# tanhuajie/Pytorch-RT1-for-Distributed-Training

Hardware: AMD Instinct MI355X
Metric: train samples/sec (whole node), RT-1 Language-Table, 1/2/4/8 MI355X (higher is better)
Workload: dtype bf16; 1 GPU; model=RT-1 (FiLM-EfficientNet-B3 + TokenLearner-8 + 8-layer transformer, 35.3M params), global_batch=128, batch_per_gpu=128, seq_len=6, parallelism=dp1, backend=hip, hipgraph=True, step=graph, graph_segments=1, tuned_library_gemms=True, full=False

## Files before the change

pytorch_rt1_for_distributed_training_amd/csrc/bindings.cpp:

```cpp
#include <algorithm>
#include <cmath>
#include <cstdlib>

#include <torch/extension.h>
#include <c10/hip/HIPStream.h>
#include <hip/hip_runtime.h>

#include "rt1_kernels.h"

namespace {

hipStream_t cur_stream() { return c10::hip::getCurrentHIPStream().stream(); }

bool sync_check() {
    static const bool on = [] {
        const char* e = std::getenv("RT1_SYNC_CHECK");
        return e != nullptr && *e != '\0' && *e != '0';
    }();
    return on;
}

void check_launch(int err, const char* what) {
    TORCH_CHECK(err == 0, what, ": HIP launch failed: ", hipGetErrorString((hipError_t)err));
    if (sync_check()) {
// ... 1522 lines not shown
          py::arg("dst"), py::arg("src"), py::arg("splits"), py::arg("sstride"));
    m.def("multi_add_", &multi_add_, "dst[i] += src[i] for many fp32 tensors, 128 per launch");
    m.def("colsum", &colsum_py, "deterministic fixed-order sum over dim 0 (fp32/bf16 in, fp32 out)");
    m.def("frame_pool", &frame_pool);
    m.def("block_tail", &block_tail);
    m.def("tail_bwd_reduce", &tail_bwd_reduce);
    m.def("stem_fwd", &stem_fwd);
    m.def("stem_bwd_weight", &stem_bwd_weight, py::arg("img"), py::arg("shift"), py::arg("dy"), py::arg("max_blocks"),
          py::arg("bn_x") = py::none(), py::arg("scale") = py::none(), py::arg("shift_bn") = py::none(),
          py::arg("mean") = py::none(), py::arg("rstd") = py::none(), py::arg("gamma") = py::none(),
          py::arg("mdz") = py::none(), py::arg("mdzx") = py::none());
    m.def("attn_fwd", &attn_fwd, py::arg("qkv"), py::arg("L"), py::arg("Kimg"), py::arg("scale"), py::arg("drop_p"),
          py::arg("seed"), py::arg("seed_dev") = py::none());
    m.def("se_bn_bwd_reduce", &se_bn_bwd_reduce);
    m.def("proj_bwd", &proj_bwd, "project-conv backward sums + dWp from (dy3, y2) per frame (skinny blocks)");
    m.def("proj_bwd_supported", &proj_bwd_supported);
    m.def("attn_keepmask", &attn_keepmask, py::arg("BH"), py::arg("S"), py::arg("drop_p"), py::arg("seed"),
          py::arg("like"), py::arg("seed_dev") = py::none());
    m.def("attn_bwd", &attn_bwd, py::arg("qkv"), py::arg("out"), py::arg("dout"), py::arg("lse"), py::arg("L"),
          py::arg("Kimg"), py::arg("scale"), py::arg("drop_p"), py::arg("seed"), py::arg("seed_dev") = py::none());
    m.def("tf_ln_fwd", &tf_ln_fwd);
    m.def("tf_ln_bwd", &tf_ln_bwd, py::arg("dy"), py::arg("x"), py::arg("mu"), py::arg("rs"), py::arg("g"),
          py::arg("dres") = py::none(), py::arg("want_bf") = false);
    m.def("tf_resid", &tf_resid, py::arg("x"), py::arg("a"), py::arg("bias"), py::arg("p"), py::arg("seed"),
          py::arg("seed_dev") = py::none(), py::arg("lg") = py::none(), py::arg("lb") = py::none(), py::arg("eps") = 1e-6);
    m.def("tf_drop_bwd", &tf_drop_bwd, py::arg("dout"), py::arg("p"), py::arg("seed"), py::arg("seed_dev") = py::none());
    m.def("pw_gemm_supported", &pw_gemm_supported);
    m.def("pw_stats_supported", &pw_stats_supported);
    m.def("add_scaled_", &add_scaled_);
    m.def("pw_bwd_supported", &pw_bwd_supported);
    m.def("pw_bwd", &pw_bwd);
    m.def("pw_bwd_z", &pw_bwd_z);
    m.def("pw_z_prep", &pw_z_prep);
    m.def("pw_gemm_bnbwd_supported", &pw_gemm_bnbwd_supported);
    m.def("pw_gemm_bnbwd", &pw_gemm_bnbwd);
    m.def("pw_tall_tail", &pw_tall_tail, py::arg("A"), py::arg("W"), py::arg("A2"), py::arg("W2"), py::arg("bias"),
          py::arg("res") = py::none(), py::arg("rmul") = py::none(), py::arg("rhw") = 1);
    m.def("pw_z_finish", &pw_z_finish);
    rt1comm::register_comm(m);
    rt1head::register_head(m);
    m.def("pw_gemm", &pw_gemm, py::arg("A"), py::arg("B"), py::arg("max_blocks"), py::arg("stats") = false,
          py::arg("scale") = py::none(), py::arg("shift") = py::none(), py::arg("gate") = py::none(),
          py::arg("hw") = 0, py::arg("store_operand") = false);
}
```

pytorch_rt1_for_distributed_training_amd/csrc/kernels/pwbwd.hip:

```cpp
#include "common.h"

using namespace rt1;

namespace {

typedef short bf16x8 __attribute__((ext_vector_type(8)));
typedef short bf16x4 __attribute__((ext_vector_type(4)));
typedef float f32x4 __attribute__((ext_vector_type(4)));
typedef __attribute__((address_space(3))) bf16x4 lds_v4;

constexpr int BLOCK = 256;
constexpr int ROWS = 64;
constexpr int PWZ_PF = 1;
constexpr int PWZ_PF_KC = 6;
constexpr int PWZ_PF_PART = 0;

template <int CE, int CIN>
struct BwdShape {
    static constexpr int KC = (CE + 31) / 32;
    static constexpr int CEP = KC * 32;
    static constexpr int NTI = (CIN + 15) / 16;
    static constexpr int CINP = NTI * 16;
    static constexpr int NTE = (CE + 15) / 16;
    static constexpr int TPW = (NTE + 3) / 4;
// ... 497 lines not shown
            if (ce >= CE) break;
            const uint2 ua = wl[((buf * 2 + 0) * ZP_CH + cl) * 8 + (ri >> 2)];
            const uint2 ub = wl[((buf * 2 + 1) * ZP_CH + cl) * 8 + (cj >> 2)];
            float a[4] = {__uint_as_float(ua.x << 16), __uint_as_float(ua.x & 0xffff0000u), __uint_as_float(ua.y << 16),
                          __uint_as_float(ua.y & 0xffff0000u)};
            const float b[4] = {__uint_as_float(ub.x << 16), __uint_as_float(ub.x & 0xffff0000u),
                                __uint_as_float(ub.y << 16), __uint_as_float(ub.y & 0xffff0000u)};
            const float s2 = k2[ce], s0 = k0[ce];
#pragma unroll
            for (int r = 0; r < 4; ++r) a[r] = i0 + r < CIN ? a[r] * s2 : (i0 + r == CIN ? s0 : 0.f);
#pragma unroll
            for (int r = 0; r < 4; ++r)
#pragma unroll
                for (int c = 0; c < 4; ++c) acc[r][c] = fmaf(a[r], b[c], acc[r][c]);
        }
    }
    __syncthreads();
#pragma unroll
    for (int r = 0; r < 4; ++r)
#pragma unroll
        for (int c = 0; c < 4; ++c) red[w][(ri + r) * 32 + cj + c] = acc[r][c];
    __syncthreads();
    const int oi = t >> 5, oj = t & 31;
    const int i = ti * 32 + oi, j = tj * 32 + oj;
    float sum = 0.f;
#pragma unroll
    for (int s = 0; s < ZP_SLICES; ++s) sum += red[s][t];
    if (j < CIN) {
        if (i < CIN) mk[(int64_t)i * CIN + j] = f2bf(sum);
        else if (i == CIN) r0[j] = sum;
    }
}

__global__ __launch_bounds__(256) void pw_z_finish_kernel(const float* __restrict__ S, int splits,
                                                          const float* __restrict__ G,
                                                          const float* __restrict__ sx, const bf16_t* __restrict__ We,
                                                          const float* __restrict__ consts, int CE, int CIN,
                                                          float* __restrict__ dWe) {
    const int64_t n = (int64_t)CE * CIN;
    const int64_t i = (int64_t)blockIdx.x * 256 + threadIdx.x;
    if (i >= n) return;
    const int ce = (int)(i / CIN), ci = (int)(i - (int64_t)ce * CIN);
    float s = S[i];
    for (int k = 1; k < splits; ++k) s += S[k * n + i];
    float a = 0.f;
#pragma unroll 8
    for (int cj = 0; cj < CIN; ++cj) a = fmaf(bf2f(We[(int64_t)ce * CIN + cj]), G[(int64_t)cj * CIN + ci], a);
    dWe[i] = consts[2 * CE + ce] * s + consts[3 * CE + ce] * a + consts[4 * CE + ce] * sx[ci];
}

#define PWBWD_SHAPES(X) X(144, 24) X(192, 32) X(288, 48)

template <int CE, int CIN>
int launch(const bf16_t* dA, const bf16_t* y, const bf16_t* x, const bf16_t* We, const float* consts, int M,
           bf16_t* dx, const bf16_t* dout, const float* fmul, int HW, float* dwp, int grid, hipStream_t st) {
    using S = BwdShape<CE, CIN>;
    if (dout)
        hipLaunchKernelGGL((pw_bwd_kernel<CE, CIN, true>), dim3(grid), dim3(BLOCK), S::lds, st, dA, y, x, We, consts,
                           M, dx, dout, fmul, HW, dwp);
    else
        hipLaunchKernelGGL((pw_bwd_kernel<CE, CIN, false>), dim3(grid), dim3(BLOCK), S::lds, st, dA, y, x, We, consts,
                           M, dx, dout, fmul, HW, dwp);
    return (int)hipGetLastError();
}

template <int CE, int CIN>
// ... 32 lines not shown
               hipStream_t st) {
#define X(A, B) if (CE == A && CIN == B) return launch<A, B>(dA, y, x, We, consts, M, dx, dout, fmul, HW, dwp, grid, st);
    PWBWD_SHAPES(X)
#undef X
    return (int)hipErrorInvalidValue;
}

int rt1_pw_bwd_z_width(int CE, int CIN) { return CE * CIN + CIN * CIN + CIN; }
int rt1_pw_bwd_z_mk_elems(int CIN) { return 2 * ((CIN + 15) / 16 * 16) * ((CIN + 31) / 32 * 32); }

int rt1_pw_bwd_z(const bf16_t* dz, const bf16_t* x, const bf16_t* We, const float* consts, int M, int CE, int CIN,
                 bf16_t* mk, float* r0, bf16_t* dx, const bf16_t* dout, const float* fmul, int HW, float* part,
                 int grid, hipStream_t st) {
    if (!rt1_pw_bwd_supported(CE, CIN) || M <= 0 || grid <= 0) return (int)hipErrorInvalidValue;
    const int CINP = (CIN + 15) / 16 * 16, KCP = (CIN + 31) / 32 * 32;
    hipLaunchKernelGGL(pw_bwd_prep_kernel, dim3((CINP * KCP + CIN + 255) / 256), dim3(256),
                       (size_t)CE * 8 + (size_t)CE * CIN * 2, st, We, consts, CE, CIN, CINP, KCP, mk, r0);
#define X(A, B) if (CE == A && CIN == B) return launch_z<A, B>(dz, x, We, consts, mk, r0, M, dx, dout, fmul, HW, part, grid, st);
    PWBWD_SHAPES(X)
#undef X
    return (int)hipErrorInvalidValue;
}

int rt1_pw_bwd_z_finish(const float* S, const bf16_t* We, const float* consts, int CE, int CIN, float* dWe,
                        hipStream_t st) {
    hipLaunchKernelGGL(pw_bwd_finish_kernel, dim3((CE * CIN + 255) / 256), dim3(256), 0, st, S, We, consts, CE, CIN,
                       dWe);
    return (int)hipGetLastError();
}

int rt1_pw_z_prep(const bf16_t* We, const float* consts, int CE, int CIN, bf16_t* wt, bf16_t* mk, float* r0,
                  hipStream_t st) {
    if (CIN <= 0 || CE <= 0) return (int)hipErrorInvalidValue;
    const int tj_n = (CIN + 31) / 32, ti_n = (CIN + 1 + 31) / 32;
    const int n_mk = ti_n * tj_n, n_wt = ((CE + 31) / 32) * tj_n;
    hipLaunchKernelGGL(pw_z_prep_kernel, dim3((unsigned)(n_mk + n_wt)), dim3(ZP_THREADS), 0, st, We, consts, CE, CIN,
                       n_mk, tj_n, wt, mk, r0);
    return (int)hipGetLastError();
}

int rt1_pw_z_finish(const float* S, int splits, const float* G, const float* sx, const bf16_t* We,
                    const float* consts, int CE, int CIN, float* dWe, hipStream_t st) {
    const int64_t n = (int64_t)CE * CIN;
    if (splits < 1) return (int)hipErrorInvalidValue;
    hipLaunchKernelGGL(pw_z_finish_kernel, dim3((unsigned)((n + 255) / 256)), dim3(256), 0, st, S, splits, G, sx, We,
                       consts, CE, CIN, dWe);
    return (int)hipGetLastError();
}

}
```

pytorch_rt1_for_distributed_training_amd/csrc/kernels/se.hip:

```cpp
#include <algorithm>
#include <cstdlib>

#include "common.h"

using namespace rt1;

namespace {

constexpr int COLS = 64, RG = 16, BLOCK = COLS * RG;
constexpr int CO_NARROW = 16;
#ifndef SE_NARROW_MAX
#define SE_NARROW_MAX 4096
#endif
__host__ __device__ constexpr int rg_of(int co) { return BLOCK / co; }

template <int NACC, int CO = COLS>
__device__ __forceinline__ void column_reduce(double (&acc)[NACC], double (*sh)[BLOCK / CO][CO]) {
    constexpr int RGN = BLOCK / CO;
    const int cl = threadIdx.x % CO, rg = threadIdx.x / CO;
#pragma unroll
    for (int a = 0; a < NACC; ++a) sh[a][rg][cl] = acc[a];
    __syncthreads();
    if (rg == 0) {
#pragma unroll
// ... 69 lines not shown
            const float g = gate[i];
            const float r = rbraw[i] * inv_hw;
            rb[i] = r;
            acc[0] += (double)(g * red[NC + i] + r * red[2 * NC + i]);
            acc[1] += (double)(g * red[3 * NC + i] + r * red[4 * NC + i]);
        }
    }
    column_reduce<2, CO>(acc, sh);
    if (rg == 0 && c < C) {
        sdz[c] = (float)acc[0];
        sdzx[c] = (float)acc[1];
        mdz[c] = (float)(acc[0] / count);
        mdzx[c] = (float)(acc[1] / count);
    }
}


constexpr int SE_BLOCK = 256;
constexpr int RD_FT = 32, RD_JT = 32, RD_KC = 64, RD_LD = RD_KC + 4;
constexpr int RM_CT = 128;
constexpr int WS_CT = 64, WS_JT = 32, WS_FC = 32, WS_NS = 8;

template <bool BWD>
__global__ NO_PACKED_FP32 __launch_bounds__(SE_BLOCK) void se_rowdot_kernel(const float* __restrict__ X, const float* __restrict__ gate,
                                                             const float* __restrict__ W, int N, int C, int S,
                                                             int kslice, float* __restrict__ part) {
    __shared__ __attribute__((aligned(16))) float xs[RD_FT][RD_LD];
    __shared__ __attribute__((aligned(16))) float ws[RD_JT][RD_LD];
    const int t = threadIdx.x;
    const int n0 = blockIdx.x * RD_FT, j0 = blockIdx.y * RD_JT, ks = blockIdx.z;
    const int kb = ks * kslice, ke = min(C, kb + kslice);
    const int fr = (t >> 4) * 2, ur = (t & 15) * 2;
    float acc[2][2] = {{0.f, 0.f}, {0.f, 0.f}};
    for (int c0 = kb; c0 < ke; c0 += RD_KC) {
        __syncthreads();
        for (int i = t; i < RD_FT * RD_KC / 4; i += SE_BLOCK) {
            const int r = i / (RD_KC / 4), q = (i % (RD_KC / 4)) * 4, n = n0 + r, c = c0 + q;
            float4 v = make_float4(0.f, 0.f, 0.f, 0.f);
            if (n < N && c < ke) {
                const int64_t o = (int64_t)n * C + c;
                v = *reinterpret_cast<const float4*>(X + o);
                if constexpr (BWD) {
                    const float4 g = *reinterpret_cast<const float4*>(gate + o);
                    v.x *= g.x * (1.f - g.x); v.y *= g.y * (1.f - g.y);
                    v.z *= g.z * (1.f - g.z); v.w *= g.w * (1.f - g.w);
                }
            }
            *reinterpret_cast<float4*>(&xs[r][q]) = v;
        }
        if constexpr (!BWD) {
            for (int i = t; i < RD_JT * RD_KC / 4; i += SE_BLOCK) {
                const int r = i / (RD_KC / 4), q = (i % (RD_KC / 4)) * 4, j = j0 + r, c = c0 + q;
                float4 v = make_float4(0.f, 0.f, 0.f, 0.f);
                if (j < S && c < ke) v = *reinterpret_cast<const float4*>(W + (int64_t)j * C + c);
                *reinterpret_cast<float4*>(&ws[r][q]) = v;
            }
        } else {
            for (int i = t; i < RD_JT * RD_KC; i += SE_BLOCK) {
                const int q = i / RD_JT, r = i % RD_JT, j = j0 + r, c = c0 + q;
                ws[r][q] = (j < S && c < ke) ? W[(int64_t)c * S + j] : 0.f;
            }
        }
        __syncthreads();
#pragma unroll 4
        for (int k = 0; k < RD_KC; k += 4) {
            const float4 x0 = *reinterpret_cast<const float4*>(&xs[fr][k]);
            const float4 x1 = *reinterpret_cast<const float4*>(&xs[fr + 1][k]);
            const float4 w0 = *reinterpret_cast<const float4*>(&ws[ur][k]);
            const float4 w1 = *reinterpret_cast<const float4*>(&ws[ur + 1][k]);
            acc[0][0] = fmaf(x0.w, w0.w, fmaf(x0.z, w0.z, fmaf(x0.y, w0.y, fmaf(x0.x, w0.x, acc[0][0]))));
            acc[0][1] = fmaf(x0.w, w1.w, fmaf(x0.z, w1.z, fmaf(x0.y, w1.y, fmaf(x0.x, w1.x, acc[0][1]))));
            acc[1][0] = fmaf(x1.w, w0.w, fmaf(x1.z, w0.z, fmaf(x1.y, w0.y, fmaf(x1.x, w0.x, acc[1][0]))));
            acc[1][1] = fmaf(x1.w, w1.w, fmaf(x1.z, w1.z, fmaf(x1.y, w1.y, fmaf(x1.x, w1.x, acc[1][1]))));
        }
    }
    float* pp = part + (int64_t)ks * N * S;
#pragma unroll
    for (int a = 0; a < 2; ++a)
#pragma unroll
        for (int b = 0; b < 2; ++b) {
            const int n = n0 + fr + a, j = j0 + ur + b;
            if (n < N && j < S) pp[(int64_t)n * S + j] = acc[a][b];
        }
}

__host__ __device__ constexpr int rm_fwd_stride(int S) { return S | 1; }

template <bool BWD, int FT>
__global__ NO_PACKED_FP32 __launch_bounds__(SE_BLOCK) void se_rowmat_kernel(const float* __restrict__ part, int KS,
                                                             const float* __restrict__ b1, const float* __restrict__ hin,
                                                             float* __restrict__ yout, const float* __restrict__ V,
                                                             const float* __restrict__ b2, float inv_hw, int N, int C,
                                                             int S, float* __restrict__ out) {
    constexpr int FPT = FT / 16;
    constexpr int NVB = 128 * RM_CT / SE_BLOCK;
    extern __shared__ __attribute__((aligned(16))) float sm[];
    const int SP = rm_fwd_stride(S);
    float* ys = sm;
    float* vt = sm + FT * S;
    const int t = threadIdx.x, n0 = blockIdx.x * FT, c0 = blockIdx.y * RM_CT;
    const int64_t NS_ = (int64_t)N * S;
    const int nv = S * RM_CT;
    const int dq = SE_BLOCK / S, dr = SE_BLOCK - dq * S, cl0 = t / S, j0 = t - cl0 * S;
    float v[NVB];
    const int vend = min(nv, (C - c0) * S);
#pragma unroll
    for (int u = 0; u < NVB; ++u) {
        const int i = u * SE_BLOCK + t;
        v[u] = 0.f;
        if constexpr (!BWD) {
            if (i < vend) v[u] = V[(int64_t)c0 * S + i];
        } else if (i < nv) {
            const int jj = i / RM_CT, c = c0 + i - jj * RM_CT;
            if (c < C) v[u] = V[(int64_t)jj * C + c];
        }
    }
    for (int base = 0; base < FT * S; base += 4 * SE_BLOCK) {
        float sum[4];
        int64_t o[4];
        bool ok[4];
#pragma unroll
        for (int u = 0; u < 4; ++u) {
            const int i = base + u * SE_BLOCK + t, r = i / S, n = n0 + r;
            sum[u] = 0.f;
            ok[u] = i < FT * S && n < N;
            o[u] = ok[u] ? (int64_t)n * S + (i - r * S) : 0;
        }
#pragma unroll 4
        for (int k = 0; k < KS; ++k) {
#pragma unroll
            for (int u = 0; u < 4; ++u)
                if (ok[u]) sum[u] += part[k * NS_ + o[u]];
        }
#pragma unroll
        for (int u = 0; u < 4; ++u) {
            const int i = base + u * SE_BLOCK + t;
            if (i >= FT * S) break;
            const int r = i / S, j = i - r * S, n = n0 + r;
            float y = 0.f;
            if (n < N) {
                const int64_t o = (int64_t)n * S + j;
                if constexpr (!BWD) {
                    const float hv = sum[u] * inv_hw + b1[j];
                    if (blockIdx.y == 0) yout[o] = hv;
                    y = silu(hv);
                } else {
                    const float x = hin[o];
                    const float sg = sigmoidf_(x);
                    y = sum[u] * (sg * (1.f + x * (1.f - sg)));
                    if (blockIdx.y == 0) yout[o] = y;
                }
            }
            ys[i] = y;
        }
    }
    {
        int cl = cl0, j = j0;
#pragma unroll
        for (int u = 0; u < NVB; ++u) {
            const int i = u * SE_BLOCK + t;
            if (i >= nv) break;
            if constexpr (!BWD) vt[cl * SP + j] = v[u];
            else vt[i] = v[u];
            j += dr;
            cl += dq;
            if (j >= S) { j -= S; ++cl; }
        }
    }
    __syncthreads();
    const int f = (t >> 4) * FPT, cq = (t & 15) * 4;
    float acc[FPT][8];
#pragma unroll
    for (int a = 0; a < FPT; ++a)
#pragma unroll
        for (int b = 0; b < 8; ++b) acc[a][b] = 0.f;
    for (int j = 0; j < S; ++j) {
        float vv[8];
        if constexpr (!BWD) {
#pragma unroll
            for (int b = 0; b < 4; ++b) {
                vv[b] = vt[(cq + b) * SP + j];
                vv[4 + b] = vt[(64 + cq + b) * SP + j];
            }
        } else {
            const float4 v4 = *reinterpret_cast<const float4*>(vt + j * RM_CT + cq);
            const float4 u4 = *reinterpret_cast<const float4*>(vt + j * RM_CT + 64 + cq);
            vv[0] = v4.x; vv[1] = v4.y; vv[2] = v4.z; vv[3] = v4.w;
            vv[4] = u4.x; vv[5] = u4.y; vv[6] = u4.z; vv[7] = u4.w;
        }
#pragma unroll
        for (int a = 0; a < FPT; ++a) {
            const float y = ys[(f + a) * S + j];
#pragma unroll
            for (int b = 0; b < 8; ++b) acc[a][b] = fmaf(y, vv[b], acc[a][b]);
        }
    }
#pragma unroll
    for (int a = 0; a < FPT; ++a) {
        const int n = n0 + f + a;
// ... 5 lines not shown
            float r[4];
#pragma unroll
            for (int b = 0; b < 4; ++b)
                r[b] = BWD ? acc[a][h * 4 + b] * inv_hw : sigmoidf_(acc[a][h * 4 + b] + b2[c + b]);
            *reinterpret_cast<float4*>(out + (int64_t)n * C + c) = make_float4(r[0], r[1], r[2], r[3]);
        }
    }
}

__global__ NO_PACKED_FP32 __launch_bounds__(SE_BLOCK) void se_wsum_part_kernel(const float* __restrict__ red,
                                                                const float* __restrict__ gate,
                                                                const float* __restrict__ h,
                                                                const float* __restrict__ dh,
                                                                const float* __restrict__ pool,
                                                                const float* __restrict__ rb, int N, int C, int S,
                                                                int nslice, float* __restrict__ pw2,
                                                                float* __restrict__ pw1, double* __restrict__ pc,
                                                                double* __restrict__ pj) {
    __shared__ __attribute__((aligned(16))) float zs[WS_FC][WS_CT];
    __shared__ __attribute__((aligned(16))) float ps[WS_FC][WS_CT];
    __shared__ __attribute__((aligned(16))) float hs[WS_FC][WS_JT];
    __shared__ __attribute__((aligned(16))) float ds[WS_FC][WS_JT];
    const int t = threadIdx.x;
    const int c0 = blockIdx.x * WS_CT, j0 = blockIdx.y * WS_JT, sl = blockIdx.z;
    const int nb = sl * nslice, ne = min(N, nb + nslice);
    const int cq = (t & 15) * 4, jp = (t >> 4) * 2;
    const int64_t NC = (int64_t)N * C;
    float a2[4][2], a1[4][2];
#pragma unroll
    for (int a = 0; a < 4; ++a) a2[a][0] = a2[a][1] = a1[a][0] = a1[a][1] = 0.f;
    double cz[4] = {0.0, 0.0, 0.0, 0.0}, c1[4] = {0.0, 0.0, 0.0, 0.0}, c2[4] = {0.0, 0.0, 0.0, 0.0};
    double jd[2] = {0.0, 0.0};
    const bool csum = blockIdx.y == 0, jsum = blockIdx.x == 0 && cq == 0;
    for (int f0 = nb; f0 < ne; f0 += WS_FC) {
        __syncthreads();
        for (int i = t; i < WS_FC * WS_CT / 4; i += SE_BLOCK) {
            const int r = i / (WS_CT / 4), q = (i % (WS_CT / 4)) * 4, n = f0 + r, c = c0 + q;
            float4 z = make_float4(0.f, 0.f, 0.f, 0.f), p = z;
            if (n < ne && c < C) {
                const int64_t o = (int64_t)n * C + c;
                const float4 d = *reinterpret_cast<const float4*>(red + o);
                const float4 g = *reinterpret_cast<const float4*>(gate + o);
                z = make_float4(d.x * g.x * (1.f - g.x), d.y * g.y * (1.f - g.y), d.z * g.z * (1.f - g.z),
                                d.w * g.w * (1.f - g.w));
                p = *reinterpret_cast<const float4*>(pool + o);
                if (csum) {
                    const float4 rr = *reinterpret_cast<const float4*>(rb + o);
                    const float4 r1 = *reinterpret_cast<const float4*>(red + NC + o);
                    const float4 r2 = *reinterpret_cast<const float4*>(red + 2 * NC + o);
                    const float4 r3 = *reinterpret_cast<const float4*>(red + 3 * NC + o);
                    const float4 r4 = *reinterpret_cast<const float4*>(red + 4 * NC + o);
                    const float gg[4] = {g.x, g.y, g.z, g.w}, rv[4] = {rr.x, rr.y, rr.z, rr.w};
                    const float v1[4] = {r1.x, r1.y, r1.z, r1.w}, v2[4] = {r2.x, r2.y, r2.z, r2.w};
                    const float v3[4] = {r3.x, r3.y, r3.z, r3.w}, v4[4] = {r4.x, r4.y, r4.z, r4.w};
                    const float zz[4] = {z.x, z.y, z.z, z.w};
#pragma unroll
                    for (int a = 0; a < 4; ++a) {
                        cz[a] += (double)zz[a];
                        c1[a] += (double)(gg[a] * v1[a] + rv[a] * v2[a]);
                        c2[a] += (double)(gg[a] * v3[a] + rv[a] * v4[a]);
                    }
                }
            }
            *reinterpret_cast<float4*>(&zs[r][q]) = z;
            *reinterpret_cast<float4*>(&ps[r][q]) = p;
        }
        for (int i = t; i < WS_FC * WS_JT; i += SE_BLOCK) {
            const int r = i / WS_JT, q = i % WS_JT, n = f0 + r, j = j0 + q;
            float hv = 0.f, dv = 0.f;
            if (n < ne && j < S) {
                const float x = h[(int64_t)n * S + j];
                hv = x * sigmoidf_(x);
                dv = dh[(int64_t)n * S + j];
            }
            hs[r][q] = hv;
            ds[r][q] = dv;
        }
        __syncthreads();
        const int fe = min(WS_FC, ne - f0);
        for (int r = 0; r < fe; ++r) {
            const float4 z = *reinterpret_cast<const float4*>(&zs[r][cq]);
            const float4 p = *reinterpret_cast<const float4*>(&ps[r][cq]);
            const float2 hv = *reinterpret_cast<const float2*>(&hs[r][jp]);
            const float2 dv = *reinterpret_cast<const float2*>(&ds[r][jp]);
            const float zz[4] = {z.x, z.y, z.z, z.w}, pp[4] = {p.x, p.y, p.z, p.w};
#pragma unroll
            for (int a = 0; a < 4; ++a) {
                a2[a][0] = fmaf(zz[a], hv.x, a2[a][0]);
                a2[a][1] = fmaf(zz[a], hv.y, a2[a][1]);
                a1[a][0] = fmaf(dv.x, pp[a], a1[a][0]);
                a1[a][1] = fmaf(dv.y, pp[a], a1[a][1]);
            }
            if (jsum) {
                jd[0] += (double)dv.x;
                jd[1] += (double)dv.y;
            }
        }
    }
    if (csum) {
        __shared__ double cred[3][16][WS_CT];
        __syncthreads();
        const int q = (t & 15) * 4, g = t >> 4;
#pragma unroll
        for (int a = 0; a < 4; ++a) {
            cred[0][g][q + a] = cz[a];
            cred[1][g][q + a] = c1[a];
// ... 215 lines not shown
```

pytorch_rt1_for_distributed_training_amd/csrc/rt1_kernels.h:

```cpp
#pragma once
#include <hip/hip_runtime.h>
#include <stdint.h>

extern "C" {

int rt1_flat_adam(float* p, const float* g, float* m, float* v, int64_t n, float lr, float beta1, float beta2,
                  float eps, float weight_decay, float step_size, float inv_sqrt_bc2, float grad_scale,
                  hipStream_t stream);
int rt1_flat_adam_dev(float* p, const float* g, float* m, float* v, int64_t n, const float* state,
                      const float* clip_state, float* ema, float* ema_state, const float* group_state,
                      const uint8_t* chunk_group, int G, float beta1, float beta2, float eps, float weight_decay,
                      float grad_scale, float one_minus_decay, int warmup, hipStream_t stream);
int rt1_lr_schedule_dev(float* state, const float* clip_state, const float* lr_base, float* group_state,
                        float* sched_state, int G, int kind, int64_t warmup, int64_t decay, double min_ratio,
                        hipStream_t stream);

int rt1_gradnorm_partials(int64_t n);
int rt1_grad_sumsq(const float* g, int64_t n, double* partials, hipStream_t stream);
int rt1_grad_clip_finalize(const double* partials, int P, float max_norm, float grad_scale, int skip_nonfinite,
                           float* clip_state, hipStream_t stream);
int rt1_buffer_guard(float* buf, float* shadow, int64_t n, const float* clip_state, hipStream_t stream);

}

// ... 200 lines not shown
int rt1_crop_resize_gather_u8(const uint8_t* raw, int64_t F, const int64_t* rows, const int* boxes, int N, int h,
                              int w, int H, int W, uint8_t* out, hipStream_t st);

int rt1_wgrad_splits(int64_t M, int Co, int Ci, int variant);
int rt1_wgrad_run(const rt1_bf16* dy, const rt1_bf16* a, int64_t M, int Co, int Ci, const float* scale,
                  const float* shift, const float* gate, int act, int hw, int splits, float* out, int variant,
                  int sums, hipStream_t st);
int rt1_wgrad_dymap(const float* dyf, const int* map, const rt1_bf16* a, int64_t M, int Co, int Ci, int splits,
                    float* out, float* dbout, int tile, hipStream_t st);

int rt1_proj_bwd_supported(int Cout, int Ce);
int rt1_proj_bwd_fsplit(int N, int HW, int Ce);
int rt1_proj_bwd_frame(const rt1_bf16* dy, const rt1_bf16* y, int N, int HW, int Cout, int Ce, const float* scale,
                       const float* shift, const float* mean, const float* rstd, const rt1_bf16* Wp, int fsplit,
                       float* G, float* R, hipStream_t st);
int rt1_proj_bwd_finalize(const float* G, const float* R, const float* gate, int N, int Cout, int Ce, int fsplit,
                          float* red, float* dW, hipStream_t st);

int rt1_pw_bwd_supported(int CE, int CIN);
int rt1_pw_bwd_grid(int M, int max_blocks);
int rt1_pw_bwd(const rt1_bf16* dA, const rt1_bf16* y, const rt1_bf16* x, const rt1_bf16* We, const float* consts,
               int M, int CE, int CIN, rt1_bf16* dx, const rt1_bf16* dout, const float* fmul, int HW, float* dwp,
               int grid, hipStream_t st);
int rt1_pw_bwd_z_width(int CE, int CIN);
int rt1_pw_bwd_z_mk_elems(int CIN);
int rt1_pw_bwd_z(const rt1_bf16* dz, const rt1_bf16* x, const rt1_bf16* We, const float* consts, int M, int CE,
                 int CIN, rt1_bf16* mk, float* r0, rt1_bf16* dx, const rt1_bf16* dout, const float* fmul, int HW,
                 float* part, int grid, hipStream_t st);
int rt1_pw_tall_tail(const rt1_bf16* A, const rt1_bf16* W, int M, int K, int N, const rt1_bf16* A2, const rt1_bf16* W2,
                     int K2, const float* bias, const rt1_bf16* res, const float* rmul, int rhw, rt1_bf16* C,
                     hipStream_t st);
int rt1_pw_z_prep(const rt1_bf16* We, const float* consts, int CE, int CIN, rt1_bf16* wt, rt1_bf16* mk, float* r0,
                  hipStream_t st);
int rt1_pw_z_finish(const float* S, int splits, const float* G, const float* sx, const rt1_bf16* We,
                    const float* consts, int CE, int CIN, float* dWe, hipStream_t st);
int rt1_pw_bwd_z_finish(const float* S, const rt1_bf16* We, const float* consts, int CE, int CIN, float* dWe,
                        hipStream_t st);

}
```

pytorch_rt1_for_distributed_training_amd/ops/backbone.py:

```python
from __future__ import annotations

import functools
import os
from dataclasses import dataclass, fields
from typing import List, Optional

import torch
import torch.nn.functional as F

from . import switches
from ._ext import load
from ..parallel.flat import defer_partials

ACT_NONE, ACT_SILU = 0, 1
MAX_BLOCKS = 2048
BF = torch.bfloat16


def _ext():
    return load()


def _mm(a: torch.Tensor, b: torch.Tensor) -> torch.Tensor:
    return torch.mm(a, b)
# ... 190 lines not shown
    x2d = x2d.contiguous()
    cfg = _WGRAD_TILE.get((x2d.shape[1], x2d.shape[1]))
    if cfg is None:
        G, sx = _ext().gram(x2d)
    else:
        variant, rows_per_split = cfg
        G, sx = _ext().gram(x2d, variant, max(1, min(2048, round(x2d.shape[0] / rows_per_split))))
    return G, sx


def gram_bn_consts(x2d: torch.Tensor, We_b: torch.Tensor, bnc: "BNCtx"):
    bn = bnc.bn
    return tuple(_ext().x_bn_stats(x2d, We_b, bn.weight, bn.bias, bn.eps, bn.momentum, bn.running_mean,
                                   bn.running_var))


def project_gemm(y2: torch.Tensor, Wp_b: torch.Tensor, sc2, sh2, gate, hw: int, bnc: "BNCtx", training: bool,
                 store_a: bool):
    Ce = y2.shape[-1]
    M2 = y2.numel() // Ce
    res = _ext().gemm(y2.view(M2, Ce), Wp_b, False, None, sc2, sh2, gate, hw, stats=training,
                      cfg=_GEMM_PROJ_TILE[(Ce, Wp_b.shape[0])], store_a=store_a)
    consts = bnc.train_consts(res[1], res[2], M2) if training else bnc.eval_consts()
    return res[0], consts, (res[-1] if store_a else None)


def _few_splits(part: torch.Tensor) -> torch.Tensor:
    return part if part.shape[0] <= 4 else _ext().colsum(part)


def expand_bwd_z_wide(dz: torch.Tensor, x: torch.Tensor, We: torch.Tensor, consts: torch.Tensor, res=None, gram=None,
                      dgrad: str = "z_wide"):
    ext = _ext()
    wt, mk, r0 = ext.pw_z_prep(We, consts)
    if dgrad == "z_gemm":
        dx = ext.gemm_tail(dz, wt, x, mk, r0, *(res or ()), cfg=_Z_GEMM_TILE.get((We.shape[0], We.shape[1]), -1))
    else:
        dx = ext.pw_tall_tail(dz, wt, x, mk, r0, *(res or ()))
    S = _few_splits(wgrad(dz, x, raw=True))
    G, sx = gram if gram is not None else gram_moments(x)
    return dx, ext.pw_z_finish(S, G, sx, We, consts)


_Z_WIDE_OFF = set()


@dataclass(frozen=True)
class BlockRoute:
    bn1: str
    se: str
    proj_fwd: str
    proj_bwd: str
    proj_dgrad: str
    dw_bwd: str
    dw_variant: int
    dw_blocks: int
    expand_bwd: str
    pw_bwd_blocks: int
    residual: str

    @property
    def zmode(self) -> bool:
        return self.expand_bwd in ("pw_bwd_z", "z_wide", "z_gemm")

    @property
    def dw_res(self) -> bool:
        return self.residual == "dw_bwd"


@functools.lru_cache(maxsize=None)
def plan_block(spec, N: int, H: int, W: int, in_bn: bool, flags: RouteFlags = FLAGS) -> BlockRoute:
    ext, f = _ext(), flags
    Cin, Ce, Cout, k, s = spec.in_ch, spec.expand_ch, spec.out_ch, spec.kernel, spec.stride
    expand = spec.expand_ratio != 1
    in_bn = in_bn and not expand
# ... 620 lines not shown
```

pytorch_rt1_for_distributed_training_amd/ops/switches.py:

```python
from __future__ import annotations

import os
from typing import Dict

DEFAULTS: Dict[str, str] = {
    "pw_tall": "1",
    "g256": "1",
    "wgrad_mfma": "1",
    "wgrad_deep": "1",
    "dw_fused": "1",
    "dw_s2_fused": "1",
    "dw_variant": "1",
    "dw_res": "1",
    "pw_pro": "1",
    "proj_bwd": "1",
    "se_fused": "1",
    "stem_in_block0": "1",
    "stem_bn_bwd": "1",
    "pw_bwd_z": "1",
    "pw_z_wide": "1",
    "z_gemm": "1",
    "xmode": "1",
    "gram_bn": "1",
    "gemm_proj": "1",
    "gemm_proj_dgrad": "1",
    "tall_res": "1",
    "gram_sx": "1",
    "tf_wgrad": "1",
    "tf_gemm": "1",
    "tf_fuse_ln": "1",
    "multi_copy": "1",
}


def _parse(spec: str) -> Dict[str, str]:
    out: Dict[str, str] = {}
    for item in filter(None, (s.strip() for s in spec.split(","))):
        name, sep, value = item.partition("=")
        name = name.strip()
        if not sep or name not in DEFAULTS:
            raise ValueError(f"RT1_AB: unknown or malformed switch {item!r}; known: {', '.join(sorted(DEFAULTS))}")
        out[name] = value.strip()
    return out


_OVERRIDES = _parse(os.environ.get("RT1_AB", ""))


def get(name: str) -> str:
    if name not in DEFAULTS:
        raise KeyError(name)
    return _OVERRIDES.get(name, DEFAULTS[name])

# ... 8 lines not shown
```

Baseline: 1447 samples/s.

## Use MFMA for z-prep Gram and hoist global loads in SE kernels

Adds an MFMA-based pw_z_prep kernel that computes the scaled We^T We Gram tile with 16x16x4 f32 MFMA over 16x16 output tiles, selected by a new default-on switch. Separately, the SE reduce and wgrad kernels now load global tiles into registers before the barrier and then store them to LDS, so load latency overlaps the sync. The SE rowmat partial-sum loop is reorganised into batched rounds with wider per-thread unrolling. These changes trade more register pressure for better latency hiding and matrix-core use in small backward kernels.

```diff
diff --git a/pytorch_rt1_for_distributed_training_amd/csrc/bindings.cpp b/pytorch_rt1_for_distributed_training_amd/csrc/bindings.cpp
--- a/pytorch_rt1_for_distributed_training_amd/csrc/bindings.cpp
+++ b/pytorch_rt1_for_distributed_training_amd/csrc/bindings.cpp
@@ -1578,6 +1578,7 @@
     m.def("pw_bwd", &pw_bwd);
     m.def("pw_bwd_z", &pw_bwd_z);
     m.def("pw_z_prep", &pw_z_prep);
+    m.def("pw_z_prep_variant", [](int64_t v) { return (int64_t)rt1_pw_z_prep_variant((int)v); });
     m.def("pw_gemm_bnbwd_supported", &pw_gemm_bnbwd_supported);
     m.def("pw_gemm_bnbwd", &pw_gemm_bnbwd);
     m.def("pw_tall_tail", &pw_tall_tail, py::arg("A"), py::arg("W"), py::arg("A2"), py::arg("W2"), py::arg("bias"),
diff --git a/pytorch_rt1_for_distributed_training_amd/csrc/kernels/pwbwd.hip b/pytorch_rt1_for_distributed_training_amd/csrc/kernels/pwbwd.hip
--- a/pytorch_rt1_for_distributed_training_amd/csrc/kernels/pwbwd.hip
+++ b/pytorch_rt1_for_distributed_training_amd/csrc/kernels/pwbwd.hip
@@ -553,6 +553,78 @@
     }
 }
 
+constexpr int ZM_T = 16, ZM_U = 12;
+
+__global__ __launch_bounds__(ZP_THREADS) void pw_z_prep_mfma_kernel(const bf16_t* __restrict__ We,
+                                                                    const float* __restrict__ consts, int CE, int CIN,
+                                                                    int n_mk, int tj_n, bf16_t* __restrict__ wt,
+                                                                    bf16_t* __restrict__ mk, float* __restrict__ r0) {
+    __shared__ float red[ZP_SLICES][ZM_T * ZM_T];
+    const int t = threadIdx.x;
+    const float* k1 = consts + 2 * CE;
+    const float* k2 = consts + 3 * CE;
+    const float* k0 = consts + 4 * CE;
+    if ((int)blockIdx.x >= n_mk) {
+        float(*tile)[33] = reinterpret_cast<float(*)[33]>(&red[0][0]);
+        const int b = blockIdx.x - n_mk;
+        const int tiles_ce = (CE + 31) / 32;
+        const int ce0 = (b % tiles_ce) * 32, ci0 = (b / tiles_ce) * 32;
+        const int tx = t & 31, ty = t >> 5;
+        const int ce = ce0 + ty, ci = ci0 + tx;
+        tile[ty][tx] = (ce < CE && ci < CIN) ? bf2f(We[(int64_t)ce * CIN + ci]) : 0.f;
+        __syncthreads();
+        const int ce2 = ce0 + tx, ci2 = ci0 + ty;
+        if (ce2 < CE && ci2 < CIN) wt[(int64_t)ci2 * CE + ce2] = f2bf(k1[ce2] * tile[tx][ty]);
+        return;
+    }
+    const int ti = blockIdx.x / tj_n, tj = blockIdx.x - ti * tj_n;
+    const int lane = t & 63, w = t >> 6;
+    const int li = lane & 15, lk = lane >> 4;
+    const int i = ti * ZM_T + li, j = tj * ZM_T + li;
+    const bool arow = i < CIN, rrow = i == CIN, bcol = j < CIN;
+    const float* asc = arow ? k2 : k0;
+    const int nk = (CE + 3) / 4;
+    f32x4 acc[4] = {{0.f, 0.f, 0.f, 0.f}, {0.f, 0.f, 0.f, 0.f}, {0.f, 0.f, 0.f, 0.f}, {0.f, 0.f, 0.f, 0.f}};
+    for (int s0 = w; s0 < nk; s0 += ZP_SLICES * ZM_U) {
+        float a[ZM_U], b[ZM_U];
+#pragma unroll
+        for (int u = 0; u < ZM_U; ++u) {
+            const int ce = (s0 + u * ZP_SLICES) * 4 + lk;
+            a[u] = b[u] = 0.f;
+            if (ce < CE) {
+                const bf16_t* row = We + (int64_t)ce * CIN;
+                if (arow) a[u] = bf2f(row[i]) * asc[ce];
+                else if (rrow) a[u] = asc[ce];
+                if (bcol) b[u] = bf2f(row[j]);
+            }
+        }
+#pragma unroll
+        for (int u = 0; u < ZM_U; ++u)
+            acc[u & 3] = __builtin_amdgcn_mfma_f32_16x16x4f32(a[u], b[u], acc[u & 3], 0, 0, 0);
+    }
+#pragma unroll
+    for (int r = 0; r < 4; ++r)
+        red[w][(lk * 4 + r) * ZM_T + li] = (acc[0][r] + acc[1][r]) + (acc[2][r] + acc[3][r]);
+    __syncthreads();
+    if (t < ZM_T * ZM_T) {
+        const int oi = ti * ZM_T + (t >> 4), oj = tj * ZM_T + (t & 15);
+        float p[ZP_SLICES];
+#pragma unroll
+        for (int s = 0; s < ZP_SLICES; ++s) p[s] = red[s][t];
+#pragma unroll
+        for (int h = ZP_SLICES / 2; h >= 1; h /= 2)
+#pragma unroll
+            for (int s = 0; s < h; ++s) p[s] = p[2 * s] + p[2 * s + 1];
+        const float sum = p[0];
+        if (oj < CIN) {
+            if (oi < CIN) mk[(int64_t)oi * CIN + oj] = f2bf(sum);
+            else if (oi == CIN) r0[oj] = sum;
+        }
+    }
+}
+
+int g_zprep_variant = 1;
+
 __global__ __launch_bounds__(256) void pw_z_finish_kernel(const float* __restrict__ S, int splits,
                                                           const float* __restrict__ G,
                                                           const float* __restrict__ sx, const bf16_t* __restrict__ We,
@@ -651,11 +723,24 @@
 int rt1_pw_z_prep(const bf16_t* We, const float* consts, int CE, int CIN, bf16_t* wt, bf16_t* mk, float* r0,
                   hipStream_t st) {
     if (CIN <= 0 || CE <= 0) return (int)hipErrorInvalidValue;
+    const int n_wt = ((CE + 31) / 32) * ((CIN + 31) / 32);
+    if (g_zprep_variant) {
+        const int tj_n = (CIN + ZM_T - 1) / ZM_T, n_mk = ((CIN + 1 + ZM_T - 1) / ZM_T) * tj_n;
+        hipLaunchKernelGGL(pw_z_prep_mfma_kernel, dim3((unsigned)(n_mk + n_wt)), dim3(ZP_THREADS), 0, st, We, consts,
+                           CE, CIN, n_mk, tj_n, wt, mk, r0);
+        return (int)hipGetLastError();
+    }
     const int tj_n = (CIN + 31) / 32, ti_n = (CIN + 1 + 31) / 32;
-    const int n_mk = ti_n * tj_n, n_wt = ((CE + 31) / 32) * tj_n;
+    const int n_mk = ti_n * tj_n;
     hipLaunchKernelGGL(pw_z_prep_kernel, dim3((unsigned)(n_mk + n_wt)), dim3(ZP_THREADS), 0, st, We, consts, CE, CIN,
                        n_mk, tj_n, wt, mk, r0);
     return (int)hipGetLastError();
+}
+
+int rt1_pw_z_prep_variant(int v) {
+    const int prev = g_zprep_variant;
+    if (v >= 0) g_zprep_variant = v ? 1 : 0;
+    return prev;
 }
 
 int rt1_pw_z_finish(const float* S, int splits, const float* G, const float* sx, const bf16_t* We,
diff --git a/pytorch_rt1_for_distributed_training_amd/csrc/kernels/se.hip b/pytorch_rt1_for_distributed_training_amd/csrc/kernels/se.hip
--- a/pytorch_rt1_for_distributed_training_amd/csrc/kernels/se.hip
+++ b/pytorch_rt1_for_distributed_training_amd/csrc/kernels/se.hip
@@ -125,33 +125,64 @@
     const int kb = ks * kslice, ke = min(C, kb + kslice);
     const int fr = (t >> 4) * 2, ur = (t & 15) * 2;
     float acc[2][2] = {{0.f, 0.f}, {0.f, 0.f}};
+    constexpr int NX = RD_FT * RD_KC / 4 / SE_BLOCK;
+    constexpr int NW = BWD ? RD_JT * RD_KC / SE_BLOCK : RD_JT * RD_KC / 4 / SE_BLOCK;
     for (int c0 = kb; c0 < ke; c0 += RD_KC) {
-        __syncthreads();
-        for (int i = t; i < RD_FT * RD_KC / 4; i += SE_BLOCK) {
+        const float4 f4z = make_float4(0.f, 0.f, 0.f, 0.f);
+        float4 lx[NX], lg[NX];
+        float4 lw4[BWD ? 1 : NW];
+        float lw[BWD ? NW : 1];
+#pragma unroll
+        for (int u = 0; u < NX; ++u) {
+            const int i = t + u * SE_BLOCK;
             const int r = i / (RD_KC / 4), q = (i % (RD_KC / 4)) * 4, n = n0 + r, c = c0 + q;
-            float4 v = make_float4(0.f, 0.f, 0.f, 0.f);
+            lx[u] = lg[u] = f4z;
             if (n < N && c < ke) {
                 const int64_t o = (int64_t)n * C + c;
-                v = *reinterpret_cast<const float4*>(X + o);
-                if constexpr (BWD) {
-                    const float4 g = *reinterpret_cast<const float4*>(gate + o);
-                    v.x *= g.x * (1.f - g.x); v.y *= g.y * (1.f - g.y);
-                    v.z *= g.z * (1.f - g.z); v.w *= g.w * (1.f - g.w);
-                }
+                lx[u] = *reinterpret_cast<const float4*>(X + o);
+                if constexpr (BWD) lg[u] = *reinterpret_cast<const float4*>(gate + o);
+            }
+        }
+        if constexpr (!BWD) {
+#pragma unroll
+            for (int u = 0; u < NW; ++u) {
+                const int i = t + u * SE_BLOCK;
+                const int r = i / (RD_KC / 4), q = (i % (RD_KC / 4)) * 4, j = j0 + r, c = c0 + q;
+                lw4[u] = f4z;
+                if (j < S && c < ke) lw4[u] = *reinterpret_cast<const float4*>(W + (int64_t)j * C + c);
+            }
+        } else {
+#pragma unroll
+            for (int u = 0; u < NW; ++u) {
+                const int i = t + u * SE_BLOCK;
+                const int q = i / RD_JT, r = i % RD_JT, j = j0 + r, c = c0 + q;
+                lw[u] = (j < S && c < ke) ? W[(int64_t)c * S + j] : 0.f;
+            }
+        }
+        __syncthreads();
+#pragma unroll
+        for (int u = 0; u < NX; ++u) {
+            const int i = t + u * SE_BLOCK;
+            const int r = i / (RD_KC / 4), q = (i % (RD_KC / 4)) * 4;
+            float4 v = lx[u];
+            if constexpr (BWD) {
+                const float4 g = lg[u];
+                v.x *= g.x * (1.f - g.x); v.y *= g.y * (1.f - g.y);
+                v.z *= g.z * (1.f - g.z); v.w *= g.w * (1.f - g.w);
             }
             *reinterpret_cast<float4*>(&xs[r][q]) = v;
         }
         if constexpr (!BWD) {
-            for (int i = t; i < RD_JT * RD_KC / 4; i += SE_BLOCK) {
-                const int r = i / (RD_KC / 4), q = (i % (RD_KC / 4)) * 4, j = j0 + r, c = c0 + q;
-                float4 v = make_float4(0.f, 0.f, 0.f, 0.f);
-                if (j < S && c < ke) v = *reinterpret_cast<const float4*>(W + (int64_t)j * C + c);
-                *reinterpret_cast<float4*>(&ws[r][q]) = v;
+#pragma unroll
+            for (int u = 0; u < NW; ++u) {
+                const int i = t + u * SE_BLOCK;
+                *reinterpret_cast<float4*>(&ws[i / (RD_KC / 4)][(i % (RD_KC / 4)) * 4]) = lw4[u];
             }
         } else {
-            for (int i = t; i < RD_JT * RD_KC; i += SE_BLOCK) {
-                const int q = i / RD_JT, r = i % RD_JT, j = j0 + r, c = c0 + q;
-                ws[r][q] = (j < S && c < ke) ? W[(int64_t)c * S + j] : 0.f;
+#pragma unroll
+            for (int u = 0; u < NW; ++u) {
+                const int i = t + u * SE_BLOCK;
+                ws[i % RD_JT][i / RD_JT] = lw[u];
             }
         }
         __syncthreads();
@@ -179,6 +210,20 @@
 
 __host__ __device__ constexpr int rm_fwd_stride(int S) { return S | 1; }
 
+template <int B, int PU>
+__device__ __forceinline__ void se_part_round(const float* __restrict__ p, int64_t stride, const int64_t (&o)[PU],
+                                              float (&sum)[PU]) {
+    float pv[B][PU];
+#pragma unroll
+    for (int kk = 0; kk < B; ++kk)
+#pragma unroll
+        for (int u = 0; u < PU; ++u) pv[kk][u] = p[kk * stride + o[u]];
+#pragma unroll
+    for (int kk = 0; kk < B; ++kk)
+#pragma unroll
+        for (int u = 0; u < PU; ++u) sum[u] += pv[kk][u];
+}
+
 template <bool BWD, int FT>
 __global__ NO_PACKED_FP32 __launch_bounds__(SE_BLOCK) void se_rowmat_kernel(const float* __restrict__ part, int KS,
                                                              const float* __restrict__ b1, const float* __restrict__ hin,
@@ -187,6 +232,7 @@
                                                              int S, float* __restrict__ out) {
     constexpr int FPT = FT / 16;
     constexpr int NVB = 128 * RM_CT / SE_BLOCK;
+    constexpr int PU = FT / 4;
     extern __shared__ __attribute__((aligned(16))) float sm[];
     const int SP = rm_fwd_stride(S);
     float* ys = sm;
@@ -208,45 +254,6 @@
             if (c < C) v[u] = V[(int64_t)jj * C + c];
         }
     }
-    for (int base = 0; base < FT * S; base += 4 * SE_BLOCK) {
-        float sum[4];
-        int64_t o[4];
-        bool ok[4];
-#pragma unroll
-        for (int u = 0; u < 4; ++u) {
-            const int i = base + u * SE_BLOCK + t, r = i / S, n = n0 + r;
-            sum[u] = 0.f;
-            ok[u] = i < FT * S && n < N;
-            o[u] = ok[u] ? (int64_t)n * S + (i - r * S) : 0;
-        }
-#pragma unroll 4
-        for (int k = 0; k < KS; ++k) {
-#pragma unroll
-            for (int u = 0; u < 4; ++u)
-                if (ok[u]) sum[u] += part[k * NS_ + o[u]];
-        }
-#pragma unroll
-        for (int u = 0; u < 4; ++u) {
-            const int i = base + u * SE_BLOCK + t;
-            if (i >= FT * S) break;
-            const int r = i / S, j = i - r * S, n = n0 + r;
-            float y = 0.f;
-            if (n < N) {
-                const int64_t o = (int64_t)n * S + j;
-                if constexpr (!BWD) {
-                    const float hv = sum[u] * inv_hw + b1[j];
-                    if (blockIdx.y == 0) yout[o] = hv;
-                    y = silu(hv);
-                } else {
-                    const float x = hin[o];
-                    const float sg = sigmoidf_(x);
-                    y = sum[u] * (sg * (1.f + x * (1.f - sg)));
-                    if (blockIdx.y == 0) yout[o] = y;
-                }
-            }
-            ys[i] = y;
-        }
-    }
     {
         int cl = cl0, j = j0;
 #pragma unroll
@@ -258,6 +265,45 @@
             j += dr;
             cl += dq;
             if (j >= S) { j -= S; ++cl; }
+        }
+    }
+    for (int base = 0; base < FT * S; base += PU * SE_BLOCK) {
+        float sum[PU], aux[PU];
+        int64_t o[PU];
+#pragma unroll
+        for (int u = 0; u < PU; ++u) {
+            const int i = base + u * SE_BLOCK + t, r = i / S, n = n0 + r;
+            const bool ok = i < FT * S && n < N;
+            sum[u] = 0.f;
+            o[u] = ok ? (int64_t)n * S + (i - r * S) : 0;
+            aux[u] = BWD ? hin[o[u]] : b1[ok ? i - r * S : 0];
+        }
+        int k = 0;
+        for (; k + 4 <= KS; k += 4) se_part_round<4, PU>(part + k * NS_, NS_, o, sum);
+        if (k + 2 <= KS) {
+            se_part_round<2, PU>(part + k * NS_, NS_, o, sum);
+            k += 2;
+        }
+        if (k < KS) se_part_round<1, PU>(part + k * NS_, NS_, o, sum);
+#pragma unroll
+        for (int u = 0; u < PU; ++u) {
+            const int i = base + u * SE_BLOCK + t;
+            if (i >= FT * S) break;
+            const int r = i / S, n = n0 + r;
+            float y = 0.f;
+            if (n < N) {
+                if constexpr (!BWD) {
+                    const float hv = sum[u] * inv_hw + aux[u];
+                    if (blockIdx.y == 0) yout[o[u]] = hv;
+                    y = silu(hv);
+                } else {
+                    const float x = aux[u];
+                    const float sg = sigmoidf_(x);
+                    y = sum[u] * (sg * (1.f + x * (1.f - sg)));
+                    if (blockIdx.y == 0) yout[o[u]] = y;
+                }
+            }
+            ys[i] = y;
         }
     }
     __syncthreads();
@@ -329,24 +375,54 @@
     double cz[4] = {0.0, 0.0, 0.0, 0.0}, c1[4] = {0.0, 0.0, 0.0, 0.0}, c2[4] = {0.0, 0.0, 0.0, 0.0};
     double jd[2] = {0.0, 0.0};
     const bool csum = blockIdx.y == 0, jsum = blockIdx.x == 0 && cq == 0;
+    constexpr int NQ = WS_FC * WS_CT / 4 / SE_BLOCK;
+    constexpr int NH = WS_FC * WS_JT / SE_BLOCK;
     for (int f0 = nb; f0 < ne; f0 += WS_FC) {
-        __syncthreads();
-        for (int i = t; i < WS_FC * WS_CT / 4; i += SE_BLOCK) {
+        const float4 f4z = make_float4(0.f, 0.f, 0.f, 0.f);
+        float4 ld[NQ], lg[NQ], lp[NQ], lr[NQ], l1[NQ], l2[NQ], l3[NQ], l4[NQ];
+        float lh[NH], ldh[NH];
+#pragma unroll
+        for (int u = 0; u < NQ; ++u) {
+            const int i = t + u * SE_BLOCK;
             const int r = i / (WS_CT / 4), q = (i % (WS_CT / 4)) * 4, n = f0 + r, c = c0 + q;
-            float4 z = make_float4(0.f, 0.f, 0.f, 0.f), p = z;
+            ld[u] = lg[u] = lp[u] = lr[u] = l1[u] = l2[u] = l3[u] = l4[u] = f4z;
             if (n < ne && c < C) {
                 const int64_t o = (int64_t)n * C + c;
-                const float4 d = *reinterpret_cast<const float4*>(red + o);
-                const float4 g = *reinterpret_cast<const float4*>(gate + o);
+                ld[u] = *reinterpret_cast<const float4*>(red + o);
+                lg[u] = *reinterpret_cast<const float4*>(gate + o);
+                lp[u] = *reinterpret_cast<const float4*>(pool + o);
+                if (csum) {
+                    lr[u] = *reinterpret_cast<const float4*>(rb + o);
+                    l1[u] = *reinterpret_cast<const float4*>(red + NC + o);
+                    l2[u] = *reinterpret_cast<const float4*>(red + 2 * NC + o);
+                    l3[u] = *reinterpret_cast<const float4*>(red + 3 * NC + o);
+                    l4[u] = *reinterpret_cast<const float4*>(red + 4 * NC + o);
+                }
+            }
+        }
+#pragma unroll
+        for (int u = 0; u < NH; ++u) {
+            const int i = t + u * SE_BLOCK;
+            const int r = i / WS_JT, q = i % WS_JT, n = f0 + r, j = j0 + q;
+            lh[u] = ldh[u] = 0.f;
+            if (n < ne && j < S) {
+                lh[u] = h[(int64_t)n * S + j];
+                ldh[u] = dh[(int64_t)n * S + j];
+            }
+        }
+        __syncthreads();
+#pragma unroll
+        for (int u = 0; u < NQ; ++u) {
+            const int i = t + u * SE_BLOCK;
+            const int r = i / (WS_CT / 4), q = (i % (WS_CT / 4)) * 4, n = f0 + r, c = c0 + q;
+            float4 z = f4z, p = f4z;
+            if (n < ne && c < C) {
+                const float4 d = ld[u], g = lg[u];
                 z = make_float4(d.x * g.x * (1.f - g.x), d.y * g.y * (1.f - g.y), d.z * g.z * (1.f - g.z),
                                 d.w * g.w * (1.f - g.w));
-                p = *reinterpret_cast<const float4*>(pool + o);
+                p = lp[u];
                 if (csum) {
-                    const float4 rr = *reinterpret_cast<const float4*>(rb + o);
-                    const float4 r1 = *reinterpret_cast<const float4*>(red + NC + o);
-                    const float4 r2 = *reinterpret_cast<const float4*>(red + 2 * NC + o);
-                    const float4 r3 = *reinterpret_cast<const float4*>(red + 3 * NC + o);
-                    const float4 r4 = *reinterpret_cast<const float4*>(red + 4 * NC + o);
+                    const float4 rr = lr[u], r1 = l1[u], r2 = l2[u], r3 = l3[u], r4 = l4[u];
                     const float gg[4] = {g.x, g.y, g.z, g.w}, rv[4] = {rr.x, rr.y, rr.z, rr.w};
                     const float v1[4] = {r1.x, r1.y, r1.z, r1.w}, v2[4] = {r2.x, r2.y, r2.z, r2.w};
                     const float v3[4] = {r3.x, r3.y, r3.z, r3.w}, v4[4] = {r4.x, r4.y, r4.z, r4.w};
@@ -362,13 +438,15 @@
             *reinterpret_cast<float4*>(&zs[r][q]) = z;
             *reinterpret_cast<float4*>(&ps[r][q]) = p;
         }
-        for (int i = t; i < WS_FC * WS_JT; i += SE_BLOCK) {
+#pragma unroll
+        for (int u = 0; u < NH; ++u) {
+            const int i = t + u * SE_BLOCK;
             const int r = i / WS_JT, q = i % WS_JT, n = f0 + r, j = j0 + q;
             float hv = 0.f, dv = 0.f;
             if (n < ne && j < S) {
-                const float x = h[(int64_t)n * S + j];
+                const float x = lh[u];
                 hv = x * sigmoidf_(x);
-                dv = dh[(int64_t)n * S + j];
+                dv = ldh[u];
             }
             hs[r][q] = hv;
             ds[r][q] = dv;
diff --git a/pytorch_rt1_for_distributed_training_amd/csrc/rt1_kernels.h b/pytorch_rt1_for_distributed_training_amd/csrc/rt1_kernels.h
--- a/pytorch_rt1_for_distributed_training_amd/csrc/rt1_kernels.h
+++ b/pytorch_rt1_for_distributed_training_amd/csrc/rt1_kernels.h
@@ -256,6 +256,7 @@
                      hipStream_t st);
 int rt1_pw_z_prep(const rt1_bf16* We, const float* consts, int CE, int CIN, rt1_bf16* wt, rt1_bf16* mk, float* r0,
                   hipStream_t st);
+int rt1_pw_z_prep_variant(int v);
 int rt1_pw_z_finish(const float* S, int splits, const float* G, const float* sx, const rt1_bf16* We,
                     const float* consts, int CE, int CIN, float* dWe, hipStream_t st);
 int rt1_pw_bwd_z_finish(const float* S, const rt1_bf16* We, const float* consts, int CE, int CIN, float* dWe,
diff --git a/pytorch_rt1_for_distributed_training_amd/ops/backbone.py b/pytorch_rt1_for_distributed_training_amd/ops/backbone.py
--- a/pytorch_rt1_for_distributed_training_amd/ops/backbone.py
+++ b/pytorch_rt1_for_distributed_training_amd/ops/backbone.py
@@ -246,6 +246,8 @@
 def expand_bwd_z_wide(dz: torch.Tensor, x: torch.Tensor, We: torch.Tensor, consts: torch.Tensor, res=None, gram=None,
                       dgrad: str = "z_wide"):
     ext = _ext()
+    if not _ZPREP_MFMA:
+        ext.pw_z_prep_variant(0)
     wt, mk, r0 = ext.pw_z_prep(We, consts)
     if dgrad == "z_gemm":
         dx = ext.gemm_tail(dz, wt, x, mk, r0, *(res or ()), cfg=_Z_GEMM_TILE.get((We.shape[0], We.shape[1]), -1))
@@ -255,6 +257,8 @@
     G, sx = gram if gram is not None else gram_moments(x)
     return dx, ext.pw_z_finish(S, G, sx, We, consts)
 
+
+_ZPREP_MFMA = switches.on("zprep_mfma")
 
 _Z_WIDE_OFF = set()
 
diff --git a/pytorch_rt1_for_distributed_training_amd/ops/switches.py b/pytorch_rt1_for_distributed_training_amd/ops/switches.py
--- a/pytorch_rt1_for_distributed_training_amd/ops/switches.py
+++ b/pytorch_rt1_for_distributed_training_amd/ops/switches.py
@@ -19,6 +19,7 @@
     "stem_bn_bwd": "1",
     "pw_bwd_z": "1",
     "pw_z_wide": "1",
+    "zprep_mfma": "1",
     "z_gemm": "1",
     "xmode": "1",
     "gram_bn": "1",
```

New measurement: 1457 samples/s, median of 6. About the same (+0.6%).
